# descriptinc/audiotools

Measured on NVIDIA H100. Metric: clips/sec (10s@44.1kHz) log-mel+LUFS pipeline, higher is better.
Workload: dtype f32

## Files before the change

audiotools_b200/csrc/lufs.cu:

```cuda
#include "b2a_common.h"
#include "iir_internal.h"

namespace b2a {
namespace lufs {

constexpr int L2 = 64;
constexpr int SEG = 32 * L2;
constexpr int CHS = L2 + 4;
constexpr int WPB = 12;
constexpr int NBUF = 2;
constexpr int BUF = 32 * CHS;
constexpr int MAX_STAGES = 2;
constexpr int TILE = 8192;

template <int NS>
struct Coef {
  float d0[NS], d1[NS], d2[NS], a1[NS], a2[NS];
};

__host__ __device__ inline size_t align256(size_t v) { return (v + 255) & ~(size_t)255; }

struct WsLayout {
  size_t bins, zeroed_bytes, zws, total;
};
// ... 266 lines not shown
#endif

template <int NS>
__global__ void __launch_bounds__(32 * WPB, 1)
kweight_energy_warp_kernel(const float* __restrict__ x, int rows, int T, int Tp, int nseg, int run_len, int n_runs,
                           int n_warm, Coef<NS> cf, const B2A_GRID_CONSTANT Tables<NS> tbv,
                           double* __restrict__ bins, int stride, int r, int nbins) {
  constexpr int D = 2 * NS;
  B2A_DYN_SMEM(smem);
  float* wins = reinterpret_cast<float*>(smem);
  __shared__ __align__(16) float s_map[L2 + 2][2 * D];
  __shared__ __align__(16) float s_mlane[32][D * D];
  __shared__ __align__(16) float s_mscan[5][D * D];
  __shared__ __align__(16) float s_mseg[D * D];
  const int tid = threadIdx.x, lane = tid & 31, warp = tid >> 5;
  for (int i = tid; i < (L2 + 2) * 2 * D; i += blockDim.x) {
    const int j = i / (2 * D), c = i - j * (2 * D);
    s_map[j][c] = c < D ? tbv.Wa[j][c] : tbv.Wlo[j][c - D];
  }
  for (int i = tid; i < 32 * D * D; i += blockDim.x) (&s_mlane[0][0])[i] = (&tbv.Mlane[0][0])[i];
  for (int i = tid; i < 5 * D * D; i += blockDim.x) (&s_mscan[0][0])[i] = (&tbv.Mscan[0][0])[i];
  if (tid < D * D) s_mseg[tid] = tbv.Mseg[tid];
  __syncthreads();
  const int total = rows * n_runs;
  float* win0 = wins + (size_t)warp * NBUF * BUF;

#pragma unroll 1
  for (int cur = (int)blockIdx.x * WPB + warp; cur < total; cur += (int)gridDim.x * WPB) {
    const int run = cur / rows, row = cur - run * rows;
    const int seg0 = run * run_len, seg1 = min(nseg, seg0 + run_len);
    const int segw = max(0, seg0 - n_warm);
    const float* xr = x + (size_t)row * (size_t)T;
    double* rb = bins + (size_t)row * (size_t)nbins;
    float carry[D];
#pragma unroll
    for (int j = 0; j < D; ++j) carry[j] = 0.f;
    stage_segment(xr, segw, T, win0, lane);
    float2 hseg = make_float2(0.f, 0.f);
    if (lane == 0) {
      const int t0 = segw * SEG;
      hseg.x = (t0 >= 2 && t0 - 2 < T) ? __ldg(xr + t0 - 2) : 0.f;
      hseg.y = (t0 >= 1 && t0 - 1 < T) ? __ldg(xr + t0 - 1) : 0.f;
    }
    cp_async_wait_all();
    __syncwarp();
    if (segw + 1 < seg1) stage_segment(xr, segw + 1, T, win0 + BUF, lane);
    float g[D];
    end_state_map<D>(win0, hseg, lane, s_map, g);
    int par = 0;
#pragma unroll 1
    for (int seg = segw; seg < seg1; ++seg, par ^= 1) {
      K2_STAMP(0);
      const float* win = win0 + par * BUF;
      const float* wnext = win0 + (par ^ 1) * BUF;
      const int t0 = seg * SEG;
#pragma unroll
      for (int k = 0; k < 5; ++k) {
        float o[D];
#pragma unroll
        for (int j = 0; j < D; ++j) o[j] = __shfl_up_sync(0xffffffffu, g[j], 1u << k);
        float t[D];
#pragma unroll
        for (int i = 0; i < D; ++i) t[i] = g[i] + row_dot<D>(s_mscan[k], i, o);
#pragma unroll
        for (int i = 0; i < D; ++i) g[i] = lane >= (1 << k) ? t[i] : g[i];
      }
      float ex[D], agg[D];
#pragma unroll
      for (int j = 0; j < D; ++j) {
        ex[j] = __shfl_up_sync(0xffffffffu, g[j], 1);
        if (lane == 0) ex[j] = 0.f;
        agg[j] = __shfl_sync(0xffffffffu, g[j], 31);
      }
      K2_STAMP(1);
      const bool energy = seg >= seg0;
      float y1[NS], y2[NS];
      {
        float st[D];
#pragma unroll
        for (int i = 0; i < D; ++i) st[i] = ex[i] + row_dot<D>(s_mlane[lane], i, carry);
#pragma unroll
        for (int s = 0; s < NS; ++s) { y1[s] = fmaf(tbv.rho[s], st[2 * s + 1], st[2 * s]); y2[s] = st[2 * s + 1]; }
      }
      const int n0 = t0 + lane * L2;
      const int nv = min(L2, max(0, Tp - n0));
      int j0 = n0 / stride, rem0 = n0 - j0 * stride;
      int b0 = 2 * j0 + (rem0 >= r ? 1 : 0);
      int end0 = (b0 & 1) ? (j0 + 1) * stride : j0 * stride + r;
      const int s1 = min(end0 - n0, L2);
      int s2 = L2, b1 = b0, b2 = b0;
      if (s1 < L2) {
        const int n1 = n0 + s1, j1 = n1 / stride, rem1 = n1 - j1 * stride;
        b1 = 2 * j1 + (rem1 >= r ? 1 : 0);
        const int end1 = (b1 & 1) ? (j1 + 1) * stride : j1 * stride + r;
        s2 = min(end1 - n0, L2);
        if (s2 < L2) {
          const int n2 = n0 + s2, j2 = n2 / stride, rem2 = n2 - j2 * stride;
          b2 = 2 * j2 + (rem2 >= r ? 1 : 0);
        }
      }
      const bool simple = (s1 >= L2) && (nv == L2);
      const bool clean = __all_sync(0xffffffffu, simple);
      {
        float cn[D];
#pragma unroll
        for (int i = 0; i < D; ++i) cn[i] = agg[i] + row_dot<D>(s_mseg, i, carry);
#pragma unroll
        for (int i = 0; i < D; ++i) carry[i] = cn[i];
      }
      K2_STAMP(2);
      cp_async_wait_all();
      __syncwarp();
      K2_STAMP(3);
      const float2 h = lane ? *reinterpret_cast<const float2*>(&win[CHS * (lane - 1) + L2 - 2]) : hseg;
      const float2 hnext = *reinterpret_cast<const float2*>(&win[CHS * 31 + L2 - 2]);
      const float4* c4 = reinterpret_cast<const float4*>(&win[CHS * lane]);
      float a0 = 0.f, a1 = 0.f, a2 = 0.f;
      float gn[D];
      if (energy && clean)
        recursion_and_map<NS, false>(cf, c4, h, y1, y2, s1, s2, nv, wnext, hnext, lane, s_map, a0, a1, a2, gn);
      else if (energy)
        recursion_and_map<NS, true>(cf, c4, h, y1, y2, s1, s2, nv, wnext, hnext, lane, s_map, a0, a1, a2, gn);
      else
        end_state_map<D>(wnext, hnext, lane, s_map, gn);
      K2_STAMP(4);
      if (energy) {
        const int blast = (s2 < L2) ? b2 : ((s1 < L2) ? b1 : b0);
        const int bf = __shfl_sync(0xffffffffu, b0, 0), bl = __shfl_sync(0xffffffffu, blast, 31);
        for (int id = bf; id <= bl; ++id) {
          const bool has = (b0 == id) || (!clean && ((s1 < L2 && b1 == id) || (s2 < L2 && b2 == id)));
          if (!__any_sync(0xffffffffu, has)) continue;
          float v = (b0 == id) ? a0 : 0.f;
          if (!clean) v += ((s1 < L2 && b1 == id) ? a1 : 0.f) + ((s2 < L2 && b2 == id) ? a2 : 0.f);
          v = warp_sum(v);
          if (lane == 0 && id < nbins) atomicAdd(rb + id, (double)v);
        }
      }
      K2_STAMP(5);
#pragma unroll
      for (int i = 0; i < D; ++i) g[i] = gn[i];
      hseg = hnext;
      __syncwarp();
      if (seg + 2 < seg1) stage_segment(xr, seg + 2, T, win0 + par * BUF, lane);
      K2_STAMP(6);
    }
  }
  cp_async_wait_all();
}

constexpr int GT = 128;

template <class T>
__device__ T block_sum(T v, T* scratch) {
  __syncthreads();
  scratch[threadIdx.x] = v;
  __syncthreads();
  for (int s = GT / 2; s > 0; s >>= 1) {
    if ((int)threadIdx.x < s) scratch[threadIdx.x] += scratch[threadIdx.x + s];
    __syncthreads();
  }
  return scratch[0];
}

struct GateParams {
  double G[8];
  float scale;
  int C, nblk, nbins, q;
};

__device__ __forceinline__ double block_loudness(const GateParams& gp, const float* z, int i) {
  double acc = 0.0;
  for (int c = 0; c < gp.C; ++c) acc += gp.G[c] * (double)z[c * gp.nblk + i];
  return -0.691 + 10.0 * log10(acc);
}

constexpr double GAMMA_A = -70.0;

struct Verdict {
  bool summed, counted;
};
__device__ __forceinline__ Verdict gate(double l, double Gamma_r) {
  return {!((l <= GAMMA_A) || (l <= Gamma_r)), (l > GAMMA_A) && (l > Gamma_r)};
}

__device__ __forceinline__ double relative_gate(const GateParams& gp, const float* z, float* mom, double* sd, int* si,
                                                int* n1t) {
  const int C = gp.C, nblk = gp.nblk;
  double sum1[8];
  for (int c = 0; c < C; ++c) sum1[c] = 0.0;
  int n1 = 0;
  for (int i = threadIdx.x; i < nblk; i += GT) {
    const double l = block_loudness(gp, z, i);
    if (mom) mom[i] = (float)l;
    if (!(l <= GAMMA_A))
      for (int c = 0; c < C; ++c) sum1[c] += (double)z[c * nblk + i];
    if (l > GAMMA_A) n1++;
  }
  *n1t = block_sum<int>(n1, si);
  double gr_acc = 0.0;
  for (int c = 0; c < C; ++c) {
    float zs = (float)block_sum<double>(sum1[c], sd);
    float zavg = zs / (float)*n1t;
    gr_acc += (double)zavg * gp.G[c];
  }
  return -0.691 + 10.0 * log10(gr_acc) - 10.0;
}

__device__ __forceinline__ double gated_energy(const GateParams& gp, const double (&sum2)[8], int n2t, double* sd) {
  double lacc = 0.0;
  for (int c = 0; c < gp.C; ++c) {
    float zs = (float)block_sum<double>(sum2[c], sd);
    float zavg = zs / (float)n2t;
    if (zavg != zavg) zavg = 0.f;
    if (zavg == INFINITY) zavg = 3.4028234663852886e38f;
    if (zavg == -INFINITY) zavg = -3.4028234663852886e38f;
    lacc += gp.G[c] * (double)zavg;
  }
  return lacc;
}

__global__ void __launch_bounds__(GT)
lufs_gate_kernel(const double* __restrict__ bins, GateParams gp, float* __restrict__ zws,
                 float* __restrict__ z_out, float* __restrict__ lufs_out, float* __restrict__ loud_out,
                 const float* __restrict__ target_db, int n_target, float* __restrict__ gain_out,
                 float* __restrict__ gr_out, float* __restrict__ mom_out) {
  __shared__ double sd[GT];
  __shared__ int si[GT];
  const int b = blockIdx.x, C = gp.C, nblk = gp.nblk, q = gp.q;
  const int tid = threadIdx.x;
  float* z = zws + (size_t)b * C * nblk;
  for (int idx = tid; idx < C * nblk; idx += GT) {
    int c = idx / nblk, i = idx - c * nblk;
    const double* rb = bins + ((size_t)b * C + c) * gp.nbins;
    double s = 0.0;
    for (int j = i; j < i + q; ++j) s += rb[2 * j] + rb[2 * j + 1];
    s += rb[2 * (i + q)];
    float zf = (float)s * gp.scale;
    z[idx] = zf;
    if (z_out) z_out[(size_t)b * C * nblk + idx] = zf;
  }
  __syncthreads();
  int n1t;
  const double Gamma_r = relative_gate(gp, z, mom_out ? mom_out + (size_t)b * nblk : nullptr, sd, si, &n1t);
  if (gr_out && tid == 0) gr_out[b] = n1t > 0 ? (float)Gamma_r : -INFINITY;
  double sum2[8];
  for (int c = 0; c < C; ++c) sum2[c] = 0.0;
  int n2 = 0;
  for (int i = tid; i < nblk; i += GT) {
    const Verdict v = gate(block_loudness(gp, z, i), Gamma_r);
    if (v.summed)
      for (int c = 0; c < C; ++c) sum2[c] += (double)z[c * nblk + i];
    if (v.counted) n2++;
  }
  int n2t = block_sum<int>(n2, si);
  const double lacc = gated_energy(gp, sum2, n2t, sd);
  if (tid == 0) {
    float lufs = (float)(-0.691 + 10.0 * log10(lacc));
    lufs_out[b] = lufs;
    float loud = fmaxf(lufs, -70.0f);
    if (loud_out) loud_out[b] = loud;
    if (gain_out) {
      float db = target_db[n_target == 1 ? 0 : b];
      float gdb = db - loud;
      gain_out[b] = expf(gdb * 0.11512925464970229f);
    }
  }
}

struct GradSos {
  float v[MAX_STAGES * 6];
  int n;
};

__global__ void __launch_bounds__(GT)
lufs_grad_gate_kernel(const float* __restrict__ zb, const float* __restrict__ lufs,
                      const float* __restrict__ grad_loud, const float* __restrict__ gain, GateParams gp, GradSos sos,
                      float* __restrict__ sos_out, int* __restrict__ kept, double* __restrict__ wt) {
  __shared__ double sd[GT];
  __shared__ int si[GT];
  const int b = blockIdx.x, C = gp.C, nblk = gp.nblk, tid = threadIdx.x;
  if (b == 0 && tid < sos.n) sos_out[tid] = sos.v[tid];
  const float* z = zb + (size_t)b * C * nblk;
  int n1t;
  const double Gamma_r = relative_gate(gp, z, nullptr, sd, si, &n1t);
  int* kb = kept + (size_t)b * (nblk + 1);
  double sum2[8];
  for (int c = 0; c < C; ++c) sum2[c] = 0.0;
  int n2 = 0, bad = 0;
  for (int i = tid; i < nblk; i += GT) {
    const Verdict v = gate(block_loudness(gp, z, i), Gamma_r);
    if (v.summed)
      for (int c = 0; c < C; ++c) sum2[c] += (double)z[c * nblk + i];
    if (v.counted) n2++;
    kb[i + 1] = v.counted ? 1 : 0;
    for (int c = 0; c < C; ++c) bad |= !isfinite(z[c * nblk + i]);
  }
  const int n2t = block_sum<int>(n2, si);
  const double E = gated_energy(gp, sum2, n2t, sd);
  const int n_bad = block_sum<int>(bad, si);
  int carry = 0;
  for (int i0 = 0; i0 < nblk; i0 += GT) {
    const int i = i0 + tid;
    __syncthreads();
    si[tid] = i < nblk ? kb[i + 1] : 0;
    __syncthreads();
    for (int o = 1; o < GT; o <<= 1) {
      const int t = tid >= o ? si[tid - o] : 0;
      __syncthreads();
      si[tid] += t;
      __syncthreads();
    }
    if (i < nblk) kb[i + 1] = carry + si[tid];
    carry += si[GT - 1];
// ... 31 lines not shown
                      const float* __restrict__ gate_r, unsigned* __restrict__ keys_ws, float* __restrict__ st_out,
                      float* __restrict__ stats_out) {
  __shared__ double s_e[MAX_C][GT + ST_STRIDES - 1];
  __shared__ unsigned s_keys[ST_SMEM_KEYS];
  __shared__ unsigned s_hist[2][256];
  __shared__ unsigned s_sel[2][2];
  __shared__ double sd[GT];
  __shared__ int si[GT];
  const int b = blockIdx.x, tid = threadIdx.x, C = sp.C, n = sp.n_st;
  unsigned* keys = n <= ST_SMEM_KEYS ? s_keys : keys_ws + (size_t)b * n;
  double pw = 0.0;
  int n1 = 0;
  for (int i0 = 0; i0 < n; i0 += GT) {
    const int m = min(GT, n - i0) + ST_STRIDES - 1;
    __syncthreads();
    for (int idx = tid; idx < C * m; idx += GT) {
      const int c = idx / m, j = idx - c * m;
      const double* e = bins + ((size_t)b * C + c) * sp.nbins + 2 * (size_t)(i0 + j);
      s_e[c][j] = e[0] + e[1];
    }
    __syncthreads();
    const int i = i0 + tid;
    if (i < n) {
      double acc = 0.0;
      for (int c = 0; c < C; ++c) {
        double e = 0.0;
        for (int k = 0; k < ST_STRIDES; ++k) e += s_e[c][tid + k];
        acc += sp.G[c] * e;
      }
      const float s = (float)(-0.691 + 10.0 * log10(acc / sp.len));
      if (st_out) st_out[(size_t)b * n + i] = s;
      keys[i] = __float_as_uint(s);
      if (s > -70.f) {
        pw += pow(10.0, ((double)s + 0.691) / 10.0);
        n1++;
      }
    }
  }
  const int n1t = block_sum<int>(n1, si);
  const double thr = -0.691 + 10.0 * log10(block_sum<double>(pw, sd) / n1t) - 20.0;
  int n2 = 0;
  for (int i = tid; i < n; i += GT) {
    const float s = __uint_as_float(keys[i]);
    const bool keep = s > -70.f && (double)s > thr;
    keys[i] = keep ? ord_key(s) : 0u;
    n2 += keep;
  }
  const int n2t = block_sum<int>(n2, si);
  unsigned pre[2] = {0u, 0u};
  unsigned rank[2] = {(unsigned)((n2t + 4) / 10), (unsigned)(((int64_t)19 * n2t - 9) / 20)};
  for (int shift = 24; n2t > 0 && shift >= 0; shift -= 8) {
    for (int i = tid; i < 2 * 256; i += GT) (&s_hist[0][0])[i] = 0u;
    __syncthreads();
    const unsigned hmask = shift == 24 ? 0u : ~0u << (shift + 8);
    unsigned cd[2] = {0u, 0u}, cn[2] = {0u, 0u};
    for (int i = tid; i < n; i += GT) {
      const unsigned k = keys[i];
      if (k == 0u) continue;
      const unsigned d = (k >> shift) & 255u;
#pragma unroll
      for (int r = 0; r < 2; ++r) {
        if ((k & hmask) != pre[r]) continue;
        if (cn[r] && d != cd[r]) {
          atomicAdd(&s_hist[r][cd[r]], cn[r]);
          cn[r] = 0u;
        }
        cd[r] = d;
        ++cn[r];
      }
    }
#pragma unroll
    for (int r = 0; r < 2; ++r)
      if (cn[r]) atomicAdd(&s_hist[r][cd[r]], cn[r]);
    __syncthreads();
    if (tid < 2) {
      const unsigned p = tid ? pre[1] : pre[0], k = tid ? rank[1] : rank[0];
      unsigned c = 0u, d = 0u;
      for (; d < 255u; ++d) {
        if (c + s_hist[tid][d] > k) break;
        c += s_hist[tid][d];
      }
      s_sel[tid][0] = p | (d << shift);
      s_sel[tid][1] = k - c;
    }
    __syncthreads();
    for (int r = 0; r < 2; ++r) { pre[r] = s_sel[r][0]; rank[r] = s_sel[r][1]; }
  }
  if (tid == 0) {
    float* o = stats_out + (size_t)b * 6;
    o[0] = lufs[b];
    o[1] = gate_r[b];
    if (n2t > 0) {
      const float lo = ord_val(pre[0]), hi = ord_val(pre[1]);
      o[2] = hi - lo; o[3] = (float)thr; o[4] = lo; o[5] = hi;
    } else {
      o[2] = 0.f; o[3] = -INFINITY; o[4] = -INFINITY; o[5] = -INFINITY;
    }
  }
}

struct Geometry {
  int K, stride, q, r, nblk, nbins, nseg;
};
static int geometry(int64_t Tp, double rate, double block_s, Geometry* g) {
  double kf = block_s * rate;
  int64_t K = (int64_t)kf;
  int64_t stride = (int64_t)(kf * 0.25);
  if (K < 1 || stride < 64) return -1;
  int64_t d = (Tp > K ? Tp : K) - K;
  int64_t nblk = (d + stride - 1) / stride + 1;
  g->K = (int)K; g->stride = (int)stride; g->q = (int)(K / stride); g->r = (int)(K % stride);
  g->nblk = (int)nblk;
  g->nbins = 2 * (int)(nblk + g->q);
  g->nseg = (int)((Tp + SEG - 1) / SEG);
  return 0;
}

template <int NS>
static int energy(const float* x, int64_t rows, int64_t T, int64_t Tp, const Geometry& g, const double* sos_h,
                  const double* stage_gain_h, const WsLayout& w, void* ws, void* stream) {
  Coef<NS> cf;
  for (int s = 0; s < NS; ++s) {
    const double* c = sos_h + 6 * s;
    B2A_REQUIRE(c[3] != 0.0, B2A_E_INVALID, "lufs: a0 == 0 in stage %d", s);
    float a0 = (float)c[3];
    float sg = (float)stage_gain_h[s];
    const float b0 = (float)c[0] / a0 * sg, b1 = (float)c[1] / a0 * sg, b2 = (float)c[2] / a0 * sg;
    cf.d0[s] = b0;
    cf.d1[s] = (float)((double)b0 + b1);
    cf.d2[s] = (float)((double)b0 + b1 + b2);
    cf.a1[s] = (float)c[4] / a0; cf.a2[s] = (float)c[5] / a0;
  }
  char* base = (char*)ws;
  B2A_CUDA_OK(cudaMemsetAsync(base, 0, w.zeroed_bytes, (cudaStream_t)stream));
#ifdef B2A_SIM
  const int64_t resident = 1;
#else
  const int64_t resident = num_sms();
#endif
  const double rho = max_pole_radius<NS>(cf);
  B2A_REQUIRE(rho < 1.0, B2A_E_UNSUPPORTED, "lufs: unstable filter (pole radius %g)", rho);
  int n_warm = 1;
  if (rho > 0.0) {
    const double n_tail = 40.0 * 0.6931471805599453 / -log(rho);
    n_warm = (int)((n_tail + SEG - 1) / SEG);
    if (n_warm < 1) n_warm = 1;
  }
  int64_t rpr = (resident * WPB) / rows;
  if (rpr < 1) rpr = 1;
  int run_len = (int)((g.nseg + rpr - 1) / rpr);
  if (run_len < 4 * n_warm) run_len = 4 * n_warm;
  if (run_len > g.nseg) run_len = g.nseg;
  const int n_runs = (g.nseg + run_len - 1) / run_len;
  Tables<NS> tb;
  build_tables<NS>(cf, &tb);
  const int64_t runs_all = rows * n_runs;
  const int64_t want = (runs_all + WPB - 1) / WPB;
  const unsigned grid = (unsigned)(want < resident ? want : resident);
  const size_t smem = (size_t)WPB * NBUF * BUF * sizeof(float);
  B2A_CUDA_OK(cudaFuncSetAttribute(kweight_energy_warp_kernel<NS>, cudaFuncAttributeMaxDynamicSharedMemorySize, (int)smem));
  B2A_LAUNCH(kweight_energy_warp_kernel<NS>, dim3(grid), dim3(32 * WPB), smem, stream, x, (int)rows, (int)T, (int)Tp,
             g.nseg, run_len, n_runs, n_warm, cf, tb, (double*)(base + w.bins), g.stride, g.r, g.nbins);
#ifdef B2A_K2_PROBE
  B2A_CUDA_OK(cudaOccupancyMaxActiveBlocksPerMultiprocessor(&g_k2_last[0], kweight_energy_warp_kernel<NS>, 32 * WPB,
                                                            smem));
  g_k2_last[1] = (int)grid;
  g_k2_last[2] = (int)smem;
#endif
  return B2A_OK;
}

static int energy_pass(const float* x, int64_t rows, int64_t T, int64_t Tp, const Geometry& g, const double* sos_h,
                       const double* stage_gain_h, int n_stage, const WsLayout& w, void* ws, void* stream) {
  if (n_stage == 1) return energy<1>(x, rows, T, Tp, g, sos_h, stage_gain_h, w, ws, stream);
  return energy<2>(x, rows, T, Tp, g, sos_h, stage_gain_h, w, ws, stream);
}

static int gate(int64_t B, int C, const Geometry& g, double rate, double block_s, const double* chan_gain_h,
                const WsLayout& w, void* ws, float* z_blocks, float* lufs_out, float* loud_out, const float* target_db,
                int n_target, float* gain_out, float* gr_out, float* mom_out, void* stream) {
  char* base = (char*)ws;
  GateParams gp;
  for (int c = 0; c < 8; ++c) gp.G[c] = c < C ? chan_gain_h[c] : 0.0;
  gp.scale = (float)(1.0 / (block_s * rate));
  gp.C = C; gp.nblk = g.nblk; gp.nbins = g.nbins; gp.q = g.q;
  B2A_LAUNCH(lufs_gate_kernel, dim3((unsigned)B), dim3(GT), 0, stream, (const double*)(base + w.bins), gp,
             (float*)(base + w.zws), z_blocks, lufs_out, loud_out, target_db, n_target, gain_out, gr_out, mom_out);
  B2A_CUDA_OK(cudaGetLastError());
  return B2A_OK;
}

static int check_input(int64_t B, int C, int64_t T, int64_t T_padded, int n_stage) {
  B2A_REQUIRE(B >= 1 && C >= 1 && T >= 1, B2A_E_INVALID, "lufs: empty input (B=%lld C=%d T=%lld)", (long long)B, C,
              (long long)T);
  B2A_REQUIRE(C <= MAX_C, B2A_E_INVALID, "lufs: at most 5 channels have BS.1770 gains (got %d)", C);
  B2A_REQUIRE(T_padded >= T, B2A_E_INVALID, "lufs: T_padded < T");
  B2A_REQUIRE(T_padded < (int64_t)2147483647 - 2 * TILE, B2A_E_UNSUPPORTED, "lufs: rows longer than 2^31 samples");
  B2A_REQUIRE(B * C * ((T_padded + TILE - 1) / TILE) < (int64_t)2147483647, B2A_E_UNSUPPORTED, "lufs: too many tiles");
  B2A_REQUIRE(n_stage >= 1 && n_stage <= MAX_STAGES, B2A_E_UNSUPPORTED,
              "lufs: %d biquad stages (1..%d supported: K-weighting has 2)", n_stage, MAX_STAGES);
  return B2A_OK;
}
static int check_geometry(int64_t T_padded, double rate, double block_s, Geometry* g) {
  B2A_REQUIRE(geometry(T_padded, rate, block_s, g) == 0, B2A_E_UNSUPPORTED,
              "lufs: gating stride int(block_s*rate/4) must be >= 64 samples (rate=%g block_s=%g)", rate, block_s);
  return B2A_OK;
}

constexpr double R128_BLOCK_S = 0.4;

static int64_t num_short_term(int64_t Tp, const Geometry& g) {
  const int64_t len = (int64_t)ST_STRIDES * g.stride;
  return Tp >= len ? (Tp - len) / g.stride + 1 : 0;
}

struct StatsWs {
  WsLayout k;
  size_t lufs, gate_r, keys, total;
};
static StatsWs stats_ws_layout(int64_t B, int C, const Geometry& g, int64_t n_st) {
  StatsWs s;
  s.k = ws_layout(B * C, g.nbins, g.nblk);
  size_t o = s.k.total;
  s.lufs = o; o = align256(o + sizeof(float) * B);
  s.gate_r = o; o = align256(o + sizeof(float) * B);
  s.keys = o; o = align256(o + sizeof(unsigned) * B * n_st);
  s.total = o;
  return s;
}

struct GradWs {
  size_t iir, wt, kept, sos, total;
};
static GradWs grad_ws_layout(int64_t B, int C, int64_t Tp, const Geometry& g) {
  GradWs w;
  size_t o = 0;
  w.iir = o; o = align256(o + b2a::iir::loudness_adjoint_workspace_bytes(B * C, Tp, MAX_STAGES));
  w.wt = o; o = align256(o + sizeof(double) * B * C);
  w.kept = o; o = align256(o + sizeof(int) * B * (g.nblk + 1));
  w.sos = o; o = align256(o + sizeof(float) * MAX_STAGES * 6);
  w.total = o;
  return w;
}

}
}

using namespace b2a::lufs;

extern "C" int64_t b2a_lufs_num_blocks(int64_t T_padded, double rate, double block_s) {
  Geometry g;
  if (T_padded < 1 || geometry(T_padded, rate, block_s, &g) != 0) return -1;
  return g.nblk;
}

extern "C" size_t b2a_lufs_workspace_bytes(int64_t B, int C, int64_t T_padded, double rate, double block_s) {
  Geometry g;
  if (B < 1 || C < 1 || T_padded < 1 || geometry(T_padded, rate, block_s, &g) != 0) return 0;
  return ws_layout(B * C, g.nbins, g.nblk).total;
}

extern "C" int b2a_lufs_f32(const float* x, int64_t B, int C, int64_t T, int64_t T_padded, double rate,
                            const double* sos_h, const double* stage_gain_h, int n_stage, double block_s,
                            const double* chan_gain_h, float* z_blocks, float* lufs_out, float* loud_out,
                            const float* target_db, int n_target, float* gain_out, void* ws, size_t ws_bytes,
                            void* stream) {
  B2A_REQUIRE(x && lufs_out && ws && sos_h && stage_gain_h && chan_gain_h, B2A_E_INVALID, "lufs: null pointer");
  int rc = check_input(B, C, T, T_padded, n_stage);
  if (rc != B2A_OK) return rc;
  B2A_REQUIRE(!gain_out || (target_db && (n_target == 1 || n_target == B)), B2A_E_INVALID,
              "lufs: gain_out needs target_db with 1 or B entries");
  Geometry g;
  rc = check_geometry(T_padded, rate, block_s, &g);
  if (rc != B2A_OK) return rc;
  const WsLayout w = ws_layout(B * C, g.nbins, g.nblk);
  B2A_REQUIRE(ws_bytes >= w.total, B2A_E_INVALID, "lufs: workspace too small (%zu < %zu)", ws_bytes, w.total);
  const int re = energy_pass(x, B * C, T, T_padded, g, sos_h, stage_gain_h, n_stage, w, ws, stream);
  if (re != B2A_OK) return re;
  return gate(B, C, g, rate, block_s, chan_gain_h, w, ws, z_blocks, lufs_out, loud_out, target_db, n_target, gain_out,
              nullptr, nullptr, stream);
}

extern "C" size_t b2a_lufs_backward_workspace_bytes(int64_t B, int C, int64_t T_padded, double rate, double block_s) {
  Geometry g;
  if (B < 1 || C < 1 || T_padded < 1 || geometry(T_padded, rate, block_s, &g) != 0) return 0;
  return grad_ws_layout(B, C, T_padded, g).total;
}

extern "C" int b2a_lufs_backward_f32(const float* grad_loud, const float* x, const float* gain, int64_t B, int C,
                                     int64_t T, int64_t T_padded, double rate, const double* sos_h,
                                     const double* stage_gain_h, int n_stage, double block_s, const double* chan_gain_h,
                                     const float* z_blocks, const float* lufs, float* grad_x, void* ws,
                                     size_t ws_bytes, void* stream) {
  B2A_REQUIRE(grad_loud && x && z_blocks && lufs && grad_x && ws && sos_h && stage_gain_h && chan_gain_h,
              B2A_E_INVALID, "lufs_backward: null pointer");
  int rc = check_input(B, C, T, T_padded, n_stage);
  if (rc != B2A_OK) return rc;
  Geometry g;
  rc = check_geometry(T_padded, rate, block_s, &g);
  if (rc != B2A_OK) return rc;
  const GradWs w = grad_ws_layout(B, C, T_padded, g);
  B2A_REQUIRE(ws_bytes >= w.total, B2A_E_INVALID, "lufs_backward: workspace too small (%zu < %zu)", ws_bytes,
              w.total);
  GradSos sos;
  sos.n = 6 * n_stage;
  for (int s = 0; s < n_stage; ++s) {
    const double* c = sos_h + 6 * s;
    B2A_REQUIRE(c[3] != 0.0, B2A_E_INVALID, "lufs_backward: a0 == 0 in stage %d", s);
// ... 78 lines not shown
```

audiotools_b200/csrc/spectral.cu:

```cuda
#include "b2a_common.h"
#include "fft_warp.cuh"
#include "grad_internal.h"
#include "spectral_internal.h"

namespace b2a {
namespace spectral {

constexpr int THREADS = 256;
constexpr int E = 16;

template <int LOG2N>
struct Plan {
  static constexpr int N = 1 << LOG2N;
  static constexpr int TPF = N / E;
  static constexpr int G = THREADS / TPF;
  static constexpr int P = (LOG2N + 3) / 4;
  static constexpr int radix(int p) {
    return (p < LOG2N / 4) ? 16 : (1 << (LOG2N % 4));
  }
  static constexpr int ns(int p) { return 1 << (4 * p); }
  static constexpr int slots(int p) { return p == 0 ? 0 : (E / radix(p)) * (radix(p) - 1); }
  static constexpr int slot_off(int p) {
    int o = 0;
    for (int i = 1; i < p; ++i) o += slots(i);
// ... 137 lines not shown
  const int hop = p.hop, n_fft = 2 * N;
  const float g = p.gain ? __ldg(p.gain + row / p.rows_per_gain) : 1.0f;
  const int ws = (n0 + p.drop_edge) * hop - N - p.pad;

  for (int i = tid; i < n_fft; i += THREADS) win[i] = __ldg(p.window + i);
  for (int i = tid; i < PL::NSLOT * TPF; i += THREADS) {
    const int slot = i / TPF, q = i - slot * TPF;
    int pass = 1;
#pragma unroll
    for (int pp = 1; pp < P; ++pp)
      if (slot >= PL::slot_off(pp)) pass = pp;
    const int R = PL::radix(pass), NS = PL::ns(pass);
    const int s = slot - PL::slot_off(pass);
    const int b = s / (R - 1), t = s - b * (R - 1) + 1;
    const int k = (q + TPF * b) & (NS - 1);
    float sn, cs;
    sincospif(-2.0f * (float)(k * t) / (float)(NS * R), &sn, &cs);
    tw[i] = make_float2(cs, sn);
  }
  for (int i = tid; i <= N / 2; i += THREADS) {
    float sn, cs;
    sincospif(-(float)i / (float)N, &sn, &cs);
    ut[i] = make_float2(cs, sn);
  }

  stage_span(p, sp, row, tile, n0, FR, ws, g);
  __syncthreads();

  const int grp = tid / TPF, q = tid - grp * TPF;
  float2* buf = bufs + grp * PL::BUF;
  float* mag = mags + grp * PL::MAG;
  const int F = N + 1;

  for (int rd = 0; rd < FR / G; ++rd) {
    const int f = rd * G + grp;
    const int n = n0 + f;
    const bool live = n < p.n_frames;
    const float* fs = sp + f * hop;

    float2 v[E];
    if ((hop & 1) == 0) {
#pragma unroll
      for (int m = 0; m < E; ++m) {
        const int e = q + TPF * m;
        const float2 s2 = *reinterpret_cast<const float2*>(fs + 2 * e);
        const float2 w2 = *reinterpret_cast<const float2*>(win + 2 * e);
        v[m] = make_float2(s2.x * w2.x, s2.y * w2.y);
      }
    } else {
#pragma unroll
      for (int m = 0; m < E; ++m) {
        const int e = q + TPF * m;
        v[m] = make_float2(fs[2 * e] * win[2 * e], fs[2 * e + 1] * win[2 * e + 1]);
      }
    }
    {
      float2 out[E];
      DFT<E, 1>::run(v, out);
#pragma unroll
      for (int t = 0; t < E; ++t) buf[buf_phys<LOG2N>(q * E + t)] = out[t];
    }
    group_sync<TPF>(grp);
    if constexpr (P >= 2) {
#pragma unroll
      for (int m = 0; m < E; ++m) v[m] = buf[buf_phys<LOG2N>(q + TPF * m)];
      group_sync<TPF>(grp);
      fft_pass<LOG2N, 1>(v, buf, tw, q);
      group_sync<TPF>(grp);
    }
    if constexpr (P >= 3) {
#pragma unroll
      for (int m = 0; m < E; ++m) v[m] = buf[buf_phys<LOG2N>(q + TPF * m)];
      group_sync<TPF>(grp);
      fft_pass<LOG2N, 2>(v, buf, tw, q);
      group_sync<TPF>(grp);
    }

    for (int k = q; k <= N / 2; k += TPF) {
      const float2 zk = buf[buf_phys<LOG2N>(k)];
      const float2 zn = buf[buf_phys<LOG2N>((N - k) & (N - 1))];
      const float2 xe = make_float2(0.5f * (zk.x + zn.x), 0.5f * (zk.y - zn.y));
      const float2 xo = make_float2(0.5f * (zk.y + zn.y), 0.5f * (zn.x - zk.x));
      const float2 tt = cmul(ut[k], xo);
      const float2 xk = cadd(xe, tt);
      const float2 d = csub(xe, tt);
      const float2 xnk = make_float2(d.x, -d.y);
      if (p.stft_out && live) {
        float2* o = p.stft_out + (size_t)row * F * p.n_frames + n;
        o[(size_t)k * p.n_frames] = xk;
        o[(size_t)(N - k) * p.n_frames] = xnk;
      }
      mag[k] = sqrtf(fmaf(xk.x, xk.x, xk.y * xk.y));
      mag[N - k] = sqrtf(fmaf(xnk.x, xnk.x, xnk.y * xnk.y));
    }
    group_sync<TPF>(grp);

    if (p.mel_out) {
      for (int m = q; m < p.n_mels; m += TPF) {
        const int lo = __ldg(p.mel_lo + m), hi = __ldg(p.mel_hi + m);
        const float* wrow = p.mel_fb + (size_t)m * F;
        float acc = 0.f;
        for (int k = lo; k < hi; ++k) acc = fmaf(__ldg(wrow + k), mag[k], acc);
        if (p.post == B2A_POST_LOG10) {
          float c = fmaxf(acc, p.post_eps);
          c = (p.post_power == 2.0f) ? c * c : powf(c, p.post_power);
          acc = log10f(c);
        } else if (p.post == B2A_POST_LN) {
          acc = logf(acc + p.post_eps);
        }
        melt[m * (FR + 1) + f] = acc;
      }
    }
    group_sync<TPF>(grp);
  }

  if (p.mel_out) {
    __syncthreads();
    const int nf = min(FR, p.n_frames - n0);
    float* o = p.mel_out + (size_t)row * p.n_mels * p.n_frames + n0;
    for (int i = tid; i < p.n_mels * FR; i += THREADS) {
      const int m = i / FR, f = i - m * FR;
      if (f < nf) o[(size_t)m * p.n_frames + f] = melt[m * (FR + 1) + f];
    }
  }
}

template <int LOG2N>
static int launch(Params& p, void* stream) {
  using PL = Plan<LOG2N>;
  p.span = (PL::FR - 1) * p.hop + p.n_fft;
  p.n_tiles = (p.n_frames + PL::FR - 1) / PL::FR;
  int o = align16(p.span * 4);
  p.off_win = o; o = align16(o + p.n_fft * 4);
  p.off_tw = o; o = align16(o + PL::NSLOT * PL::TPF * 8 + 16);
  p.off_ut = o; o = align16(o + (PL::N / 2 + 1) * 8);
  p.off_buf = o; o = align16(o + PL::G * PL::BUF * 8);
  p.off_mag = o; o = align16(o + PL::G * PL::MAG * 4);
  p.off_mel = o; o = align16(o + (p.mel_out ? p.n_mels * (PL::FR + 1) * 4 : 0));
  p.smem_bytes = o;
  B2A_REQUIRE(o <= 227 * 1024, B2A_E_UNSUPPORTED,
              "spectral: n_fft=%d hop=%d n_mels=%d needs %d bytes of shared memory (> 227 KB)", p.n_fft, p.hop,
              p.n_mels, o);
  B2A_REQUIRE((int64_t)p.rows * p.n_tiles < (int64_t)2147483647, B2A_E_UNSUPPORTED, "spectral: grid too large");
  B2A_CUDA_OK(cudaFuncSetAttribute(spectral_kernel<LOG2N>, cudaFuncAttributeMaxDynamicSharedMemorySize, o));
  B2A_LAUNCH(spectral_kernel<LOG2N>, dim3((unsigned)(p.rows * p.n_tiles)), dim3(THREADS), (size_t)o, stream, p);
  B2A_CUDA_OK(cudaGetLastError());
  return B2A_OK;
}



#ifdef B2A_K1_PROBE
__device__ unsigned long long* g_k1_probe;
#define K1_PROBE_TILES 64
#define K1_STAMP(k)                                                                                   \
  do {                                                                                                \
    if (g_k1_probe && lane == 0 && it_probe < K1_PROBE_TILES)                                         \
      g_k1_probe[(((size_t)blockIdx.x * 8 + warp) * K1_PROBE_TILES + it_probe) * 11 + (k)] = clock64(); \
  } while (0)
#else
#define K1_STAMP(k) do { } while (0)
#endif

template <int LOG2N, int MODE>
__global__ void __launch_bounds__(256, 2) spectral_warp_kernel(Params p) {
  using PL = WPlan<LOG2N>;
  constexpr bool STAGED = (MODE == 1), DIRECT = (MODE == 2);
  constexpr int N = PL::N, LPF = PL::LPF, FPW = PL::FPW, G = PL::G, FR = PL::FR;
  static_assert(FR == G && FR % 8 == 0, "one round per tile: the |X| slot of a frame is its index in the tile");
  B2A_DYN_SMEM(smem);
  float* sp = reinterpret_cast<float*>(smem);
  float* win = reinterpret_cast<float*>(smem + p.off_win);
  float2* tw = reinterpret_cast<float2*>(smem + p.off_tw);
  float2* ut = reinterpret_cast<float2*>(smem + p.off_ut);
  float* xbs = reinterpret_cast<float*>(smem + p.off_buf);
  float* mpk = reinterpret_cast<float*>(smem + p.off_mpk);
  int4* mseg = reinterpret_cast<int4*>(smem + p.off_mseg);

  const int tid = threadIdx.x, lane = tid & 31, warp = tid >> 5;
  const int hop = p.hop, n_fft = 2 * N, F = N + 1;
  const int l = lane & (LPF - 1);
  const int fw = lane / LPF;
  const int total_tiles = p.rows * p.n_tiles;

  int t = blockIdx.x;
  __shared__ __align__(8) unsigned long long s_bar;
  if (tid == 0) mbar_init(&s_bar, 1);
  __syncthreads();
  bool by_tma;
  unsigned tma_parity = 0;
  {
    const int row = t / p.n_tiles, tile = t - row * p.n_tiles;
    by_tma = stage_span_async(p, sp, row,
                              (tile * FR + p.drop_edge) * hop + p.origin + (p.row_origin ? __ldg(p.row_origin + row) : 0),
                              &s_bar);
  }
  for (int i = tid; i < n_fft; i += 256) win[i] = 0.5f * __ldg(p.window + i);
  for (int i = tid; i < G * p.xb_stride; i += 256) xbs[i] = 0.f;
  warp_fft_tables<LOG2N, PL::NUT>(tw, ut);
  const bool packed = p.mel_out && p.mel_packed_len > 0;
  __shared__ int s_clamp;
  if (packed) {
    for (int m = tid; m < p.n_mels; m += 256) {
      const int lo4 = __ldg(p.mel_lo + m) & ~3;
      int n4 = (((__ldg(p.mel_hi + m) + 3) & ~3) - lo4) >> 2;
      mseg[m] = make_int4(0, lo4, n4 < 0 ? 0 : n4, 0);
    }
    __syncthreads();
    if (tid == 0) {
      int run = 0, reach = 0;
      for (int w = 0; w < 8; ++w)
        for (int i = 0; 4 * (w + 8 * i) < p.n_mels; ++i) {
          int mx = 0;
          for (int j = 0; j < 4; ++j) { const int m = 4 * (w + 8 * i) + j; if (m < p.n_mels) mx = max(mx, mseg[m].z); }
          mx = (mx + 1) & ~1;
          for (int j = 0; j < 4; ++j) {
            const int m = 4 * (w + 8 * i) + j;
            if (m < p.n_mels) { mseg[m].x = run; mseg[m].w = mx; run += mx; reach = max(reach, mseg[m].y + 4 * mx); }
          }
        }
      s_clamp = reach > PL::XB;
    }
    __syncthreads();
    for (int m = warp; m < p.n_mels; m += 8) {
      const int4 sg = mseg[m];
      const float* wrow = p.mel_fb + (size_t)m * F;
      for (int i = lane; i < 4 * sg.w; i += 32) {
        const int k = sg.y + i;
        mpk[4 * sg.x + i] = (i < 4 * sg.z && k < F) ? __ldg(wrow + k) : 0.f;
      }
    }
  }

  float* xb = xbs + (warp * FPW + fw) * p.xb_stride;
  const int src_lane = partner_lane<LPF>(lane);

#ifdef B2A_K1_PROBE
  int it_probe = 0;
#endif
  bool first = true;
#pragma unroll 1
  for (; t < total_tiles; t += gridDim.x) {
    const int row = t / p.n_tiles, tile = t - row * p.n_tiles;
    const int n0 = tile * FR;
    const int ws = (n0 + p.drop_edge) * hop + p.origin + (p.row_origin ? __ldg(p.row_origin + row) : 0);
    const float g = p.gain ? __ldg(p.gain + row / p.rows_per_gain) : 1.0f;
    const float ga = fabsf(g);
    K1_STAMP(0);
    if (by_tma) { mbar_wait(&s_bar, tma_parity); tma_parity ^= 1u; }
    K1_STAMP(1);
#ifdef B2A_SIM
    __syncthreads();
#else
    if (!by_tma || first) __syncthreads();
#endif
    first = false;
    K1_STAMP(2);
    if (p.y_out) writeback_scaled(p, sp, row, tile, n0, FR, ws, g);
    K1_STAMP(3);

#pragma unroll 1
    for (int rd = 0; rd < FR / G; ++rd) {
      const int f = rd * G + warp * FPW + fw;
      const int n = n0 + f;
      const bool live = n < p.n_frames;
      const float* fs = sp + f * hop;

      float2 z[32];
      load_frame<LOG2N>(fs, win, hop, z, l);
      K1_STAMP(4);
      if (rd == FR / G - 1) {
        __syncthreads();
        const int tn = t + gridDim.x;
        by_tma = false;
        if (tn < total_tiles) {
          const int rown = tn / p.n_tiles, tilen = tn - rown * p.n_tiles;
          by_tma = stage_span_async(
              p, sp, rown, (tilen * FR + p.drop_edge) * hop + p.origin + (p.row_origin ? __ldg(p.row_origin + rown) : 0),
              &s_bar);
        }
      }
      K1_STAMP(5);
      warp_fft<LOG2N, true>(z, xb, tw, l);

      const float2 u0 = ut[l];
      float2* so = (DIRECT && p.stft_out) ? p.stft_out + (size_t)row * F * p.n_frames + n : nullptr;
#pragma unroll
      for (int m = 0; m < 16; ++m) {
        const float2 zk = z[m];
        float2 zn;
        zn.x = __shfl_sync(0xffffffffu, z[31 - m].x, src_lane);
        zn.y = __shfl_sync(0xffffffffu, z[31 - m].y, src_lane);
        if (l == 0) zn = z[(32 - m) & 31];
        const int k = l + LPF * m;
        const float2 xe = add2(zk, make_float2(zn.x, -zn.y));
        const float2 xo = add2(make_float2(zk.y, -zk.x), make_float2(zn.y, zn.x));
        const float2 w = untangle_twiddle_m<LOG2N>(ut, u0, l, m);
        const float2 xk = fma2(bcast2(w.x), xo, fma2(make_float2(-w.y, w.y), make_float2(xo.y, xo.x), xe));
        const float2 d = fma2(bcast2(2.0f), xe, neg2(xk));
        if constexpr (STAGED) {
          float2* xc = reinterpret_cast<float2*>(xb);
          xc[k] = make_float2(g * xk.x, g * xk.y);
          xc[N - k] = make_float2(g * d.x, -g * d.y);
        } else {
          if constexpr (DIRECT) {
            if (so && live) {
              so[(size_t)k * p.n_frames] = make_float2(g * xk.x, g * xk.y);
              so[(size_t)(N - k) * p.n_frames] = make_float2(g * d.x, -g * d.y);
            }
          }
          xb[k] = fast_sqrt(fmaf(xk.x, xk.x, xk.y * xk.y));
          xb[N - k] = fast_sqrt(fmaf(d.x, d.x, d.y * d.y));
        }
      }
      if (l == 0) {
        const float2 zh = make_float2(2.0f * z[16].x, 2.0f * z[16].y);
        if constexpr (STAGED) {
          reinterpret_cast<float2*>(xb)[N / 2] = make_float2(g * zh.x, -g * zh.y);
        } else {
          if constexpr (DIRECT) {
            if (so && live) so[(size_t)(N / 2) * p.n_frames] = make_float2(g * zh.x, -g * zh.y);
          }
          xb[N / 2] = fast_sqrt(fmaf(zh.x, zh.x, zh.y * zh.y));
          xb[N + 1] = 0.f; xb[N + 2] = 0.f; xb[N + 3] = 0.f;
        }
      }
      __syncwarp();

    }
    K1_STAMP(6);

    const int nf = min(FR, p.n_frames - n0);
    float* mo = p.mel_out ? p.mel_out + (size_t)row * p.n_mels * p.n_frames + n0 : nullptr;
    if (p.mel_out) {
      __syncthreads();
      K1_STAMP(7);
      const int fl = lane & 7, jq = lane >> 3;
      const float lscale = p.post_power * 0.30102999566398120f;
      if (packed) {
        const float4* mpk4 = reinterpret_cast<const float4*>(mpk);
        for (int fc = 0; fc < FR; fc += 8) {
          const int f = fc + fl;
          const float* xf = xbs + f * p.xb_stride;
          if (!s_clamp) {
            for (int mm = 4 * warp + jq; mm < p.n_mels; mm += 32) {
              const int4 sg = mseg[mm];
              const float4* w4 = mpk4 + sg.x;
              const float4* v4 = reinterpret_cast<const float4*>(xf + sg.y);
              float2 a01 = make_float2(0.f, 0.f), a23 = a01;
              for (int it = 0; it < sg.w; it += 2) {
                const float4 wa = w4[it], wb = w4[it + 1], va = v4[it], vb = v4[it + 1];
                a01 = fma2(make_float2(wa.x, wa.y), make_float2(va.x, va.y), a01);
                a23 = fma2(make_float2(wb.x, wb.y), make_float2(vb.x, vb.y), a23);
                a01 = fma2(make_float2(wa.z, wa.w), make_float2(va.z, va.w), a01);
                a23 = fma2(make_float2(wb.z, wb.w), make_float2(vb.z, vb.w), a23);
              }
              float acc = ((a01.x + a01.y) + (a23.x + a23.y)) * ga;
              if (p.post == B2A_POST_LOG10) acc = lscale * fast_log2(fmaxf(acc, p.post_eps));
              else if (p.post == B2A_POST_LN) acc = logf(acc + p.post_eps);
              if (f < nf) mo[(size_t)mm * p.n_frames + f] = acc;
            }
          } else {
            const int lim = PL::XB - 4;
            for (int mm = 4 * warp + jq; mm < p.n_mels; mm += 32) {
              const int4 sg = mseg[mm];
              const float4* w4 = mpk4 + sg.x;
              float a0 = 0.f, a1 = 0.f;
              for (int it = 0; it < sg.w; ++it) {
                const float4 w = w4[it];
                const float4 v = *reinterpret_cast<const float4*>(xf + min(sg.y + 4 * it, lim));
                a0 = fmaf(w.x, v.x, a0); a1 = fmaf(w.y, v.y, a1);
                a0 = fmaf(w.z, v.z, a0); a1 = fmaf(w.w, v.w, a1);
              }
              float acc = (a0 + a1) * ga;
              if (p.post == B2A_POST_LOG10) acc = lscale * fast_log2(fmaxf(acc, p.post_eps));
              else if (p.post == B2A_POST_LN) acc = logf(acc + p.post_eps);
              if (f < nf) mo[(size_t)mm * p.n_frames + f] = acc;
            }
          }
        }
      } else {
        for (int fc = 0; fc < FR; fc += 8) {
          const int f = fc + fl;
// ... 101 lines not shown
  B2A_REQUIRE(pad >= 0 && right_pad >= 0 && drop_edge >= 0, B2A_E_INVALID, "%s: negative padding", who);
  B2A_REQUIRE(pad_mode >= 0 && pad_mode <= 2, B2A_E_UNSUPPORTED, "%s: pad mode %d", who, pad_mode);
  const int64_t Lp = T + 2 * (int64_t)pad + right_pad;
  B2A_REQUIRE(n_fft / 2 < Lp, B2A_E_INVALID, "%s: n_fft/2 (%d) must be < padded length (%lld)", who, n_fft / 2,
              (long long)Lp);
  B2A_REQUIRE(pad_mode != B2A_PAD_REFLECT || (pad + right_pad) < T || (pad + right_pad) == 0, B2A_E_INVALID,
              "%s: reflect padding (%d) must be < signal length (%lld)", who, pad + right_pad, (long long)T);
  *n_frames = b2a_stft_num_frames(T, n_fft, hop, pad, right_pad, drop_edge);
  B2A_REQUIRE(*n_frames >= 1, B2A_E_INVALID, "%s: no frames", who);
  return B2A_OK;
}

}
}

extern "C" int64_t b2a_stft_num_frames(int64_t T, int n_fft, int hop, int pad, int right_pad, int drop_edge) {
  if (T < 1 || n_fft < 2 || hop < 1 || pad < 0 || right_pad < 0 || drop_edge < 0) return -1;
  int64_t n = 1 + (T + 2 * (int64_t)pad + right_pad - (n_fft & 1)) / hop - 2 * (int64_t)drop_edge;
  return n;
}

extern "C" int b2a_stft_route(int n_fft, int hop, int inverse) {
  if (n_fft < 2 || hop < 1 || (inverse && hop > n_fft)) return B2A_ROUTE_NONE;
  if ((n_fft & (n_fft - 1)) == 0) {
    if (n_fft >= (inverse ? 64 : 32) && n_fft <= (inverse ? 2048 : 4096)) return B2A_ROUTE_FFT;
    if (n_fft >= 4096 && n_fft <= 32768) return B2A_ROUTE_LARGE;
  }
  return n_fft <= 8192 ? B2A_ROUTE_DENSE : B2A_ROUTE_NONE;
}

static int spectral_fft(const float* x, int64_t rows, int64_t T, int n_fft, int hop, const float* window, int pad,
                        int right_pad, int pad_mode, int drop_edge, const float* gain, int rows_per_gain, float* y_out,
                        const float* mel_fb, const int32_t* mel_lo, const int32_t* mel_hi, int n_mels,
                        int mel_packed_len, int post, float post_eps, float post_power, float* mel_out,
                        float* stft_out, void* stream) {
  using namespace b2a::spectral;
  B2A_REQUIRE(x && window, B2A_E_INVALID, "spectral: null x/window");
  B2A_REQUIRE(mel_out || stft_out, B2A_E_INVALID, "spectral: neither mel_out nor stft_out requested");
  B2A_REQUIRE(rows >= 1 && T >= 1, B2A_E_INVALID, "spectral: empty input");
  B2A_REQUIRE(T < (int64_t)1 << 30, B2A_E_UNSUPPORTED, "spectral: rows longer than 2^30 samples");
  B2A_REQUIRE(n_fft >= 32 && n_fft <= 4096 && (n_fft & (n_fft - 1)) == 0, B2A_E_UNSUPPORTED,
              "spectral: window_length must be a power of two in [32, 4096] (got %d)", n_fft);
  B2A_REQUIRE(hop >= 1, B2A_E_INVALID, "spectral: hop_length must be >= 1");
  int64_t nfr;
  const int rc = check_framing("spectral", T, n_fft, hop, pad, right_pad, pad_mode, drop_edge, &nfr);
  if (rc != B2A_OK) return rc;
  B2A_REQUIRE(!y_out || (pad == 0 && right_pad == 0 && drop_edge == 0), B2A_E_UNSUPPORTED,
              "spectral: y_out needs pad == right_pad == drop_edge == 0");
  B2A_REQUIRE(!gain || rows_per_gain >= 1, B2A_E_INVALID, "spectral: rows_per_gain");
  B2A_REQUIRE(!mel_out || (mel_fb && mel_lo && mel_hi && n_mels >= 1), B2A_E_INVALID, "spectral: mel arguments");
  B2A_REQUIRE(post >= 0 && post <= 2, B2A_E_INVALID, "spectral: post-op %d", post);
  Params p;
  memset(&p, 0, sizeof(p));
  p.x = x; p.window = window; p.gain = gain; p.y_out = y_out;
  p.mel_fb = mel_fb; p.mel_lo = mel_lo; p.mel_hi = mel_hi; p.mel_out = mel_out;
  p.stft_out = reinterpret_cast<float2*>(stft_out);
  p.rows = (int)rows; p.T = (int)T; p.n_fft = n_fft; p.hop = hop; p.pad = pad; p.right_pad = right_pad;
  p.pad_mode = pad_mode; p.drop_edge = drop_edge; p.n_frames = (int)nfr; p.n_mels = n_mels;
  p.mel_packed_len = (mel_out && mel_packed_len > 0) ? mel_packed_len : 0;
  p.center = 1; p.origin = -(n_fft / 2) - pad; p.row_origin = nullptr;
  p.rows_per_gain = gain ? rows_per_gain : 1; p.post = post; p.post_eps = post_eps; p.post_power = post_power;
  switch (n_fft) {
    case 32: return launch<4>(p, stream);
    case 64: return launch_warp<5>(p, stream);
    case 128: return launch_warp<6>(p, stream);
    case 256: return launch_warp<7>(p, stream);
    case 512: return launch_warp<8>(p, stream);
    case 1024: return launch_warp<9>(p, stream);
    case 2048: return launch_warp<10>(p, stream);
    case 4096: return launch<11>(p, stream);
  }
  return b2a::fail(B2A_E_UNSUPPORTED, "spectral: n_fft %d", n_fft);
}

extern "C" size_t b2a_spectral_workspace_bytes(int64_t rows, int64_t T, int n_fft, int hop, int pad, int right_pad,
                                                int drop_edge, int stft_scratch, int scaled_scratch) {
  const int r = b2a_stft_route(n_fft, hop, 0);
  const int64_t nfr = b2a_stft_num_frames(T, n_fft, hop, pad, right_pad, drop_edge);
  if (rows < 1 || nfr < 1 || r == B2A_ROUTE_NONE || r == B2A_ROUTE_FFT) return 0;
  size_t bytes = 0;
  if (stft_scratch) bytes += (size_t)rows * (size_t)(n_fft / 2 + 1) * (size_t)nfr * 2 * sizeof(float);
  if (scaled_scratch) bytes += (size_t)rows * (size_t)T * sizeof(float);
  return bytes;
}

static int spectral_materialised(int route, const float* x, int64_t rows, int64_t T, int n_fft, int hop,
                                 const float* window, const float* matrix, int pad, int right_pad, int pad_mode,
                                 int drop_edge, const float* gain, int rows_per_gain, float* y_out,
                                 const float* mel_fb, const int32_t* mel_lo, const int32_t* mel_hi, int n_mels,
                                 int post, float post_eps, float post_power, float* mel_out, float* stft_out,
                                 void* ws, size_t ws_bytes, void* stream) {
  B2A_REQUIRE(mel_out || stft_out, B2A_E_INVALID, "spectral: neither mel_out nor stft_out requested");
  int64_t nfr;
  int rc = b2a::spectral::check_framing(route == B2A_ROUTE_LARGE ? "stft_large" : "stft_dense", T, n_fft, hop, pad,
                                        right_pad, pad_mode, drop_edge, &nfr);
  if (rc != B2A_OK) return rc;
  const size_t need = b2a_spectral_workspace_bytes(rows, T, n_fft, hop, pad, right_pad, drop_edge, !stft_out,
                                                   gain && !y_out);
  B2A_REQUIRE(ws_bytes >= need && (ws || need == 0), B2A_E_INVALID, "spectral: workspace too small");
  B2A_REQUIRE(((uintptr_t)ws & 7) == 0, B2A_E_INVALID, "spectral: workspace must be 8-byte aligned");
  const int F = n_fft / 2 + 1;
  char* scratch = static_cast<char*>(ws);
  float* stft = stft_out;
  if (!stft) {
    stft = reinterpret_cast<float*>(scratch);
    scratch += (size_t)rows * F * (size_t)nfr * 2 * sizeof(float);
  }
  if (gain) {
    B2A_REQUIRE(rows_per_gain >= 1 && rows % rows_per_gain == 0, B2A_E_INVALID, "spectral: rows_per_gain");
    float* scaled = y_out ? y_out : reinterpret_cast<float*>(scratch);
    rc = b2a_gain_f32(x, scaled, rows / rows_per_gain, rows_per_gain * T, gain, stream);
    if (rc != B2A_OK) return rc;
    x = scaled;
  }
  rc = route == B2A_ROUTE_LARGE
           ? b2a::large::stft(x, rows, T, n_fft, hop, window, pad, right_pad, pad_mode, drop_edge, stft, stream)
           : b2a::dft::stft(x, rows, T, n_fft, hop, matrix, pad, right_pad, pad_mode, drop_edge, stft, stream);
  if (rc != B2A_OK || !mel_out) return rc;
  return b2a::dft::mel_from_stft(stft, rows, F, nfr, mel_fb, mel_lo, mel_hi, n_mels, post, post_eps, post_power,
                                 mel_out, stream);
}

extern "C" int b2a_spectral_f32(const float* x, int64_t rows, int64_t T, int n_fft, int hop, const float* window,
                                const float* matrix, int pad, int right_pad, int pad_mode, int drop_edge,
                                const float* gain, int rows_per_gain, float* y_out, const float* mel_fb,
                                const int32_t* mel_lo, const int32_t* mel_hi, int n_mels, int mel_packed_len, int post,
                                float post_eps, float post_power, float* mel_out, float* stft_out, void* ws,
                                size_t ws_bytes, void* stream) {
  const int route = b2a_stft_route(n_fft, hop, 0);
  if (route == B2A_ROUTE_FFT)
    return spectral_fft(x, rows, T, n_fft, hop, window, pad, right_pad, pad_mode, drop_edge, gain, rows_per_gain, y_out,
                        mel_fb, mel_lo, mel_hi, n_mels, mel_packed_len, post, post_eps, post_power, mel_out, stft_out,
                        stream);
  if (route == B2A_ROUTE_LARGE || route == B2A_ROUTE_DENSE)
    return spectral_materialised(route, x, rows, T, n_fft, hop, window, matrix, pad, right_pad, pad_mode, drop_edge,
                                 gain, rows_per_gain, y_out, mel_fb, mel_lo, mel_hi, n_mels, post, post_eps, post_power,
                                 mel_out, stft_out, ws, ws_bytes, stream);
  return b2a::fail(B2A_E_UNSUPPORTED,
                   "spectral: n_fft=%d hop=%d (hop >= 1; powers of two up to 32768, any other length up to 8192)",
                   n_fft, hop);
}

extern "C" int b2a_spectral_tc_enable(int on) {
  if (on == 0) return 0;
  return b2a::fail(B2A_E_UNSUPPORTED,
                   "spectral_tc_enable: the tensor-core spectral kernel was removed; the FP32 kernel runs every launch");
}

#ifdef B2A_K1_PROBE
extern "C" int b2a_k1_probe_set(void* buf) {
  B2A_CUDA_OK(cudaMemcpyToSymbol(b2a::spectral::g_k1_probe, &buf, sizeof(buf)));
  return B2A_OK;
}
extern "C" int b2a_k1_probe_tiles() { return K1_PROBE_TILES; }
extern "C" void b2a_k1_probe_last(int* out) {
  for (int i = 0; i < 3; ++i) out[i] = b2a::spectral::g_k1_last[i];
}
#endif
```

Measured before the change: 100,400.

## Parallelize spectral mel-table prologue, warp-shuffle block_sum, cache LUFS host tables

The spectral kernel prologue now builds its packed mel segment table with a warp-wide prefix scan instead of a single serial thread. It fills the packed filterbank with all threads writing float4s through a per-slot mel index map, rather than one warp per mel row. The LUFS block_sum finishes with warp shuffles instead of a log-step shared-memory loop, which drops several barriers. The host-side IIR tables are cached in thread_local storage keyed on the coefficients, so they are not rebuilt every call. A probe that records per-warp entry timestamps is also added under an ifdef.

```diff
diff --git a/audiotools_b200/csrc/lufs.cu b/audiotools_b200/csrc/lufs.cu
--- a/audiotools_b200/csrc/lufs.cu
+++ b/audiotools_b200/csrc/lufs.cu
@@ -442,13 +442,20 @@
 
 template <class T>
 __device__ T block_sum(T v, T* scratch) {
+  static_assert(GT == 128, "two shared-memory levels, then one warp");
+  const int tid = threadIdx.x;
   __syncthreads();
-  scratch[threadIdx.x] = v;
+  scratch[tid] = v;
   __syncthreads();
-  for (int s = GT / 2; s > 0; s >>= 1) {
-    if ((int)threadIdx.x < s) scratch[threadIdx.x] += scratch[threadIdx.x + s];
-    __syncthreads();
-  }
+  if (tid < 64) scratch[tid] += scratch[tid + 64];
+  __syncthreads();
+  if (tid < 32) {
+    T a = scratch[tid] + scratch[tid + 32];
+#pragma unroll
+    for (int s = 16; s > 0; s >>= 1) a += __shfl_down_sync(0xffffffffu, a, s);
+    if (tid == 0) scratch[0] = a;
+  }
+  __syncthreads();
   return scratch[0];
 }
 
@@ -786,8 +793,14 @@
   if (run_len < 4 * n_warm) run_len = 4 * n_warm;
   if (run_len > g.nseg) run_len = g.nseg;
   const int n_runs = (g.nseg + run_len - 1) / run_len;
-  Tables<NS> tb;
-  build_tables<NS>(cf, &tb);
+  thread_local Coef<NS> tb_cf;
+  thread_local Tables<NS> tb;
+  thread_local bool tb_built = false;
+  if (!tb_built || memcmp(&tb_cf, &cf, sizeof(cf)) != 0) {
+    build_tables<NS>(cf, &tb);
+    tb_cf = cf;
+    tb_built = true;
+  }
   const int64_t runs_all = rows * n_runs;
   const int64_t want = (runs_all + WPB - 1) / WPB;
   const unsigned grid = (unsigned)(want < resident ? want : resident);
diff --git a/audiotools_b200/csrc/spectral.cu b/audiotools_b200/csrc/spectral.cu
--- a/audiotools_b200/csrc/spectral.cu
+++ b/audiotools_b200/csrc/spectral.cu
@@ -313,6 +313,7 @@
 
 #ifdef B2A_K1_PROBE
 __device__ unsigned long long* g_k1_probe;
+__device__ unsigned long long* g_k1_entry;
 #define K1_PROBE_TILES 64
 #define K1_STAMP(k)                                                                                   \
   do {                                                                                                \
@@ -344,6 +345,9 @@
   const int fw = lane / LPF;
   const int total_tiles = p.rows * p.n_tiles;
 
+#ifdef B2A_K1_PROBE
+  if (g_k1_entry && lane == 0) g_k1_entry[(size_t)blockIdx.x * 8 + warp] = clock64();
+#endif
   int t = blockIdx.x;
   __shared__ __align__(8) unsigned long long s_bar;
   if (tid == 0) mbar_init(&s_bar, 1);
@@ -357,39 +361,82 @@
                               &s_bar);
   }
   for (int i = tid; i < n_fft; i += 256) win[i] = 0.5f * __ldg(p.window + i);
-  for (int i = tid; i < G * p.xb_stride; i += 256) xbs[i] = 0.f;
-  warp_fft_tables<LOG2N, PL::NUT>(tw, ut);
   const bool packed = p.mel_out && p.mel_packed_len > 0;
-  __shared__ int s_clamp;
-  if (packed) {
+  if (packed)
     for (int m = tid; m < p.n_mels; m += 256) {
       const int lo4 = __ldg(p.mel_lo + m) & ~3;
       int n4 = (((__ldg(p.mel_hi + m) + 3) & ~3) - lo4) >> 2;
       mseg[m] = make_int4(0, lo4, n4 < 0 ? 0 : n4, 0);
     }
+  for (int i = tid; i < G * p.xb_stride; i += 256) xbs[i] = 0.f;
+  warp_fft_tables<LOG2N, PL::NUT>(tw, ut);
+  __shared__ int s_clamp, s_slots;
+  if (packed) {
     __syncthreads();
-    if (tid == 0) {
+    if (warp == 0) {
+      const int Q = (p.n_mels + 3) >> 2;
       int run = 0, reach = 0;
-      for (int w = 0; w < 8; ++w)
-        for (int i = 0; 4 * (w + 8 * i) < p.n_mels; ++i) {
-          int mx = 0;
-          for (int j = 0; j < 4; ++j) { const int m = 4 * (w + 8 * i) + j; if (m < p.n_mels) mx = max(mx, mseg[m].z); }
-          mx = (mx + 1) & ~1;
+      for (int k0 = 0; k0 < Q; k0 += 32) {
+        const int k = k0 + lane;
+        int q = -1;
+        for (int w = 0, s = 0; w < 8 && w < Q; ++w) {
+          const int c = (Q - w + 7) >> 3;
+          if (k >= s && k < s + c) q = w + 8 * (k - s);
+          s += c;
+        }
+        int mx = 0, nv = 0;
+        if (q >= 0)
+          for (int j = 0; j < 4; ++j) { const int m = 4 * q + j; if (m < p.n_mels) { mx = max(mx, mseg[m].z); ++nv; } }
+        mx = (mx + 1) & ~1;
+        int incl = nv * mx;
+        for (int o = 1; o < 32; o <<= 1) {
+          const int v = __shfl_up_sync(0xffffffffu, incl, o);
+          if (lane >= o) incl += v;
+        }
+        int off = run + incl - nv * mx;
+        if (q >= 0)
           for (int j = 0; j < 4; ++j) {
-            const int m = 4 * (w + 8 * i) + j;
-            if (m < p.n_mels) { mseg[m].x = run; mseg[m].w = mx; run += mx; reach = max(reach, mseg[m].y + 4 * mx); }
+            const int m = 4 * q + j;
+            if (m < p.n_mels) { mseg[m].x = off; mseg[m].w = mx; off += mx; reach = max(reach, mseg[m].y + 4 * mx); }
           }
-        }
-      s_clamp = reach > PL::XB;
+        run += __shfl_sync(0xffffffffu, incl, 31);
+      }
+      for (int o = 16; o > 0; o >>= 1) reach = max(reach, __shfl_xor_sync(0xffffffffu, reach, o));
+      if (lane == 0) {
+        s_clamp = reach > PL::XB;
+        s_slots = run;
+      }
     }
     __syncthreads();
-    for (int m = warp; m < p.n_mels; m += 8) {
+    int* slot_m = reinterpret_cast<int*>(mpk);
+    for (int m = tid; m < p.n_mels; m += 256) {
       const int4 sg = mseg[m];
-      const float* wrow = p.mel_fb + (size_t)m * F;
-      for (int i = lane; i < 4 * sg.w; i += 32) {
-        const int k = sg.y + i;
-        mpk[4 * sg.x + i] = (i < 4 * sg.z && k < F) ? __ldg(wrow + k) : 0.f;
-      }
+      for (int j = 0; j < sg.w; ++j) slot_m[4 * (sg.x + j)] = m;
+    }
+    __syncthreads();
+    const int n_slots = s_slots;
+    for (int f0 = tid; f0 < n_slots; f0 += 4 * 256) {
+      int ms[4];
+#pragma unroll
+      for (int j = 0; j < 4; ++j) ms[j] = f0 + 256 * j < n_slots ? slot_m[4 * (f0 + 256 * j)] : -1;
+      float4 v[4];
+#pragma unroll
+      for (int j = 0; j < 4; ++j) {
+        float e[4] = {0.f, 0.f, 0.f, 0.f};
+        if (ms[j] >= 0) {
+          const int4 sg = mseg[ms[j]];
+          const float* wrow = p.mel_fb + (size_t)ms[j] * F;
+#pragma unroll
+          for (int c = 0; c < 4; ++c) {
+            const int i = 4 * (f0 + 256 * j - sg.x) + c, k = sg.y + i;
+            e[c] = (i < 4 * sg.z && k < F) ? __ldg(wrow + k) : 0.f;
+          }
+        }
+        v[j] = make_float4(e[0], e[1], e[2], e[3]);
+      }
+#pragma unroll
+      for (int j = 0; j < 4; ++j)
+        if (ms[j] >= 0) reinterpret_cast<float4*>(mpk)[f0 + 256 * j] = v[j];
     }
   }
 
@@ -797,6 +844,10 @@
   B2A_CUDA_OK(cudaMemcpyToSymbol(b2a::spectral::g_k1_probe, &buf, sizeof(buf)));
   return B2A_OK;
 }
+extern "C" int b2a_k1_probe_set_entry(void* buf) {
+  B2A_CUDA_OK(cudaMemcpyToSymbol(b2a::spectral::g_k1_entry, &buf, sizeof(buf)));
+  return B2A_OK;
+}
 extern "C" int b2a_k1_probe_tiles() { return K1_PROBE_TILES; }
 extern "C" void b2a_k1_probe_last(int* out) {
   for (int i = 0; i < 3; ++i) out[i] = b2a::spectral::g_k1_last[i];
```

Result: no change. 102,100, median of 6 (+1.7%).
